# AuburnSounds/audio-formats

Measured on AMD Instinct MI355X. Metric: decoded samples/sec (batched MP3+OGG+FLAC) at 1/2/4/8 MI355X vs CPU ref, higher is better.
Workload: dtype f32 (MP3, Vorbis, CELT) + int32 (FLAC)

## Files before the change

audio-formats_amd/csrc/afg_api.hip:

```cpp
#include "afg_common.h"

#include <atomic>
#include <cstdlib>
#include <string>

namespace afg {

static thread_local char g_err[512] = "";

void set_error(const char *fmt, ...)
{
    va_list ap;
    va_start(ap, fmt);
    vsnprintf(g_err, sizeof(g_err), fmt, ap);
    va_end(ap);
}

int require_device()
{
    int n = 0;
    hipError_t e = hipGetDeviceCount(&n);
    if (e != hipSuccess || n <= 0) {
        set_error("no HIP device available (%s); this library has no CPU fallback",
                  e == hipSuccess ? "device count 0" : hipGetErrorString(e));
        return AFG_ERR_NO_DEVICE;
    }
    int dev = 0;
    AFG_HIP_CHECK(hipGetDevice(&dev));
    hipDeviceProp_t prop;
    AFG_HIP_CHECK(hipGetDeviceProperties(&prop, dev));
    if (std::strncmp(prop.gcnArchName, "gfx950", 6) != 0) {
        set_error("device %d is %s; kernels are built for gfx950 (MI355X) only", dev, prop.gcnArchName);
        return AFG_ERR_NO_DEVICE;
    }
    return AFG_OK;
}

int device_slot(int *dev, const char *who)
{
    *dev = 0;
    AFG_HIP_CHECK(hipGetDevice(dev));
    if (*dev < 0 || *dev >= AFG_MAX_DEVICES) {
        set_error("%s: device index %d does not fit this library's per-device tables (AFG_MAX_DEVICES = %d)", who, *dev,
                  AFG_MAX_DEVICES);
        return AFG_ERR_INVALID;
    }
    return AFG_OK;
}

static std::atomic<int> g_numeric_mode{ -1 };

int numeric_mode()
{
    const int m = g_numeric_mode.load(std::memory_order_relaxed);
    if (m >= 0) return m;
    const char *e = getenv("AFG_NUMERIC");
    if (e && !strcmp(e, "exact")) return AFG_NUMERIC_EXACT;
    return AFG_NUMERIC_TOLERANCE;
}

static std::atomic<long> g_dev_option[kDevCount] = { { -1 }, { -1 }, { -1 }, { -1 }, { -1 }, { -1 }, { -1 }, { -1 }, { -1 }, { -1 }, { -1 }, { -1 }, { -1 }, { -1 }, { -1 }, { -1 } };
static const char *const k_dev_option_name[kDevCount] = { "celt_path", "celt_de_seq", "celt_de_duo", "celt_seg_recs", "celt_whole_frames",
                                                          "vorbis_single", "mp3_chunks", "mp3_float_upload", "vorbis_host_floor",
                                                          "flac_host_res32", "vorbis_seg_packets", "batch_groups", "stage_chunk_samples", "resample_scratch_bytes",
                                                          "mel_scratch_bytes", "trim_scratch_bytes" };

long dev_option(DevOption which) { return g_dev_option[which].load(std::memory_order_relaxed); }

int DeviceArray::upload(const void *host, size_t nbytes)
{
    release();
    if (nbytes == 0) return AFG_OK;
    hipError_t e = hipMalloc(&ptr, nbytes);
    if (e != hipSuccess) {
        ptr = nullptr;
        set_error("hipMalloc(%zu) failed: %s", nbytes, hipGetErrorString(e));
        return e == hipErrorOutOfMemory ? AFG_ERR_OOM : AFG_ERR_HIP;
    }
    bytes = nbytes;
    AFG_HIP_CHECK(hipMemcpy(ptr, host, nbytes, hipMemcpyHostToDevice));
    return AFG_OK;
}

void DeviceArray::release()
{
    if (ptr && owned) (void)hipFree(ptr);
    ptr = nullptr;
    bytes = 0;
    owned = true;
}

}

extern "C" {

int afg_abi_version(void) { return AFG_ABI_VERSION; }

const char *afg_status_string(int status)
{
    switch (status) {
    case AFG_OK: return "ok";
    case AFG_ERR_INVALID: return "invalid argument";
    case AFG_ERR_NO_DEVICE: return "no usable gfx950 device";
    case AFG_ERR_HIP: return "HIP runtime error";
    case AFG_ERR_OOM: return "out of memory";
    case AFG_ERR_UNSUPPORTED: return "unsupported";
    default: return "unknown status";
    }
}

const char *afg_last_error(void) { return afg::g_err; }

int afg_get_numeric_mode(void) { return afg::numeric_mode(); }

int afg_dev_option(const char *name, int value)
{
    for (int i = 0; name && i < afg::kDevCount; i++)
        if (!strcmp(name, afg::k_dev_option_name[i])) {
            afg::g_dev_option[i].store(value < 0 ? -1 : value, std::memory_order_relaxed);
            return AFG_OK;
        }
    afg::set_error("afg_dev_option: no option named '%s'", name ? name : "(null)");
    return AFG_ERR_INVALID;
}

int afg_set_numeric_mode(int mode)
{
    if (mode != AFG_NUMERIC_EXACT && mode != AFG_NUMERIC_TOLERANCE && mode != AFG_NUMERIC_FROM_ENV) {
        afg::set_error("afg_set_numeric_mode: unknown mode %d", mode);
        return AFG_ERR_INVALID;
    }
    const int prev = afg::numeric_mode();
    afg::g_numeric_mode.store(mode, std::memory_order_relaxed);
    return prev;
}

int afg_device_count(void)
{
    int n = 0;
    hipError_t e = hipGetDeviceCount(&n);
    if (e != hipSuccess) {
        afg::set_error("hipGetDeviceCount failed: %s", hipGetErrorString(e));
        return e == hipErrorNoDevice ? 0 : AFG_ERR_HIP;
    }
    return n;
}

int afg_device_name(int device, char *buf, size_t buflen)
{
    if (!buf || buflen == 0) return AFG_ERR_INVALID;
    hipDeviceProp_t prop;
    AFG_HIP_CHECK(hipGetDeviceProperties(&prop, device));
    snprintf(buf, buflen, "%s (%s, %d CUs)", prop.name, prop.gcnArchName, prop.multiProcessorCount);
    return AFG_OK;
}

int afg_device_malloc(void **d_ptr, size_t bytes)
{
    if (!d_ptr) return AFG_ERR_INVALID;
    *d_ptr = nullptr;
    if (int rc = afg::require_device()) return rc;
    hipError_t e = hipMalloc(d_ptr, bytes ? bytes : 1);
    if (e != hipSuccess) {
        afg::set_error("hipMalloc(%zu) failed: %s", bytes, hipGetErrorString(e));
        return e == hipErrorOutOfMemory ? AFG_ERR_OOM : AFG_ERR_HIP;
    }
    return AFG_OK;
}

int afg_device_free(void *d_ptr)
{
    if (d_ptr) AFG_HIP_CHECK(hipFree(d_ptr));
    return AFG_OK;
}

int afg_memcpy_h2d(void *d_dst, const void *src, size_t bytes, void *hip_stream)
{
    AFG_HIP_CHECK(hipMemcpyAsync(d_dst, src, bytes, hipMemcpyHostToDevice, (hipStream_t)hip_stream));
    return AFG_OK;
}

int afg_memcpy_d2h(void *dst, const void *d_src, size_t bytes, void *hip_stream)
{
    AFG_HIP_CHECK(hipMemcpyAsync(dst, d_src, bytes, hipMemcpyDeviceToHost, (hipStream_t)hip_stream));
    return AFG_OK;
}

namespace {
typedef float probe_f4 __attribute__((ext_vector_type(4)));
__global__ __launch_bounds__(256) void copy_probe_kernel(const probe_f4 *__restrict__ in, probe_f4 *__restrict__ out, size_t n)
{
    const size_t i = (size_t)blockIdx.x * 256 + threadIdx.x;
    if (i < n) __builtin_nontemporal_store(__builtin_nontemporal_load(in + i), out + i);
}
}

namespace {
__global__ __launch_bounds__(256) void lds_fill_kernel(uint32_t word, uint32_t *sink)
{
    extern __shared__ uint32_t lds_words[];
    for (uint32_t i = threadIdx.x; i < 160u * 1024u / 4u; i += 256) lds_words[i] = word;
    __syncthreads();
    if (sink && lds_words[(threadIdx.x * 97u) % (160u * 1024u / 4u)] != word) *sink = 1;
}
}

int afg_lds_fill_probe_hip(uint32_t word, void *hip_stream)
{
    if (int rc = afg::require_device()) return rc;
    static uint32_t *sink = nullptr;
    if (!sink) AFG_HIP_CHECK(hipMalloc(&sink, 256));
    AFG_HIP_CHECK(hipFuncSetAttribute((const void *)lds_fill_kernel, hipFuncAttributeMaxDynamicSharedMemorySize, 160 * 1024));
    hipLaunchKernelGGL(lds_fill_kernel, dim3(256 * 16), dim3(256), 160 * 1024, (hipStream_t)hip_stream, word, sink);
    AFG_HIP_CHECK(hipGetLastError());
    return AFG_OK;
}

int afg_copy_probe_hip(void *d_dst, const void *d_src, size_t bytes, void *hip_stream)
{
    if (!d_dst || !d_src || (bytes & 15) || (((uintptr_t)d_dst | (uintptr_t)d_src) & 15)) {
        afg::set_error("afg_copy_probe_hip: pointers and size must be 16-byte aligned");
        return AFG_ERR_INVALID;
    }
    if (int rc = afg::require_device()) return rc;
    const size_t n = bytes / 16, blocks = (n + 255) / 256;
    if (blocks == 0) return AFG_OK;
    if (blocks > 0x7fffffffull) {
        afg::set_error("afg_copy_probe_hip: at most 2^31 blocks of 4 KiB per call");
        return AFG_ERR_INVALID;
    }
    hipLaunchKernelGGL(copy_probe_kernel, dim3((uint32_t)blocks), dim3(256), 0, (hipStream_t)hip_stream,
                       (const probe_f4 *)d_src, (probe_f4 *)d_dst, n);
    AFG_HIP_CHECK(hipGetLastError());
    return AFG_OK;
}

int afg_stream_synchronize(void *hip_stream)
{
    AFG_HIP_CHECK(hipStreamSynchronize((hipStream_t)hip_stream));
    return AFG_OK;
}

}
```

audio-formats_amd/csrc/afg_common.h:

```cpp
#pragma once
#include <hip/hip_runtime.h>
#include <cstdarg>
#include <cstdint>
#include <cstdio>
#include <cstring>

#include "../../include/afg.h"

namespace afg {

void set_error(const char *fmt, ...);

int require_device();

#define AFG_MAX_DEVICES 64
int device_slot(int *dev, const char *who);

int numeric_mode();

enum DevOption { kDevCeltPath, kDevCeltDeSeq, kDevCeltDeDuo, kDevCeltSegRecs, kDevCeltWholeFrames, kDevVorbisSingle,
                 kDevMp3Chunks, kDevMp3FloatUpload, kDevVorbisHostFloor, kDevFlacHostRes32, kDevVorbisSegPackets, kDevBatchGroups, kDevStageChunkSamples, kDevResampleScratchBytes, kDevMelScratchBytes, kDevTrimScratchBytes, kDevCount };
long dev_option(DevOption which);

#define AFG_HIP_CHECK(expr)                                                              \
    do {                                                                                 \
        hipError_t e__ = (expr);                                                         \
        if (e__ != hipSuccess) {                                                         \
            ::afg::set_error("%s failed: %s (%s:%d)", #expr, hipGetErrorString(e__),     \
                             __FILE__, __LINE__);                                        \
            return AFG_ERR_HIP;                                                          \
        }                                                                                \
    } while (0)

struct PlanArena {
    uint8_t *host = nullptr, *dev = nullptr;
    size_t cap = 0, used = 0;
    hipStream_t stream = nullptr;
};

int mp3_plan_create_at(afg_mp3_plan **plan, uint32_t n_streams, const uint32_t *granules, const uint8_t *channels,
                       const uint64_t *blk_base, uint32_t seg_granules, PlanArena *arena = nullptr);

void mp3_launch_tolerance(uint32_t n_segs, const void *d_segs, const void *d_streams, const float *d_coef,
                          const uint32_t *d_flags, float *d_pcm, float *d_state, hipStream_t stream);

int vorbis_plan_create_at(afg_vorbis_plan **plan, uint32_t n_streams, const uint32_t *packets, const uint8_t *channels,
                          const uint16_t *blocksize0, const uint16_t *blocksize1, const uint8_t *pflags,
                          const uint64_t *spec_base, uint32_t seg_packets);

int collate_launch(const afg_collate_span *h_spans, uint64_t n_spans, const afg_collate_span *d_spans, uint64_t n_tiles,
                   const float *d_in, uint64_t in_floats, float *d_out, uint64_t out_floats, hipStream_t stream);

int resample_launch(const afg_resample_row *h_rows, uint64_t n_rows, const afg_resample_row *d_rows, uint64_t n_tiles,
                    const float *d_in, uint64_t in_floats, const float *d_taps, uint64_t taps_floats, float *d_out,
                    uint64_t out_floats, hipStream_t stream);

int melspec_launch(const afg_mel_row *h_rows, uint64_t n_rows, const afg_mel_row *d_rows, uint64_t n_tiles, const afg_mel_params *params,
                   const float *d_in, uint64_t in_floats, const float *d_basis, uint64_t basis_floats, const float *d_filters,
                   uint64_t filters_floats, float *d_out, uint64_t out_floats, hipStream_t stream);

int melspec_fft_launch(const afg_mel_row *h_rows, uint64_t n_rows, const afg_mel_row *d_rows, uint64_t n_tiles, const afg_mel_params *params,
                       const float *d_in, uint64_t in_floats, const float *d_table, uint64_t table_floats, const float *d_filters,
                       uint64_t filters_floats, float *d_out, uint64_t out_floats, hipStream_t stream);
bool mel_fft_n_ok(uint32_t n_fft);

int normalize_launch(const afg_norm_group *h_groups, uint64_t n_groups, const afg_norm_group *d_groups, uint64_t n_tiles,
                     const afg_norm_params *params, const float *d_in, uint64_t in_floats, float *d_out, uint64_t out_floats,
                     void *d_partials, afg_norm_stats *d_stats, hipStream_t stream);

int cepstra_launch(const afg_cep_row *h_rows, uint64_t n_rows, const afg_cep_row *d_rows, uint64_t n_tiles, const afg_cep_params *params,
                   const float *d_in, uint64_t in_floats, const float *d_dct, uint64_t dct_floats, float *d_out, uint64_t out_floats,
                   hipStream_t stream);

int trim_launch(const afg_trim_group *h_groups, uint64_t n_groups, const afg_trim_group *d_groups, uint64_t n_blocks, uint64_t n_tiles,
                const afg_trim_params *params, const float *d_in, uint64_t in_floats, float *d_out, uint64_t out_floats, double *d_blocks,
                afg_trim_region *d_regions, hipStream_t stream);

struct DeviceArray {
    void *ptr = nullptr;
    size_t bytes = 0;
    bool owned = true;
    int upload(const void *host, size_t nbytes);
    void release();
};

}
```

audio-formats_amd/csrc/mp3_transform.hip:

```cpp
#define AFG_MP3_FMA 0
#define AFG_MP3_KERNEL mp3_transform_kernel
#include "mp3_kernel.h"

#include <vector>

struct afg_mp3_plan {
    uint32_t n_streams = 0;
    uint32_t n_segs = 0;
    uint64_t blocks = 0;
    afg::DeviceArray d_segs, d_streams;
};

extern "C" {

int afg_mp3_plan_create(afg_mp3_plan **plan, uint32_t n_streams, const uint32_t *granules,
                        const uint8_t *channels, uint32_t seg_granules)
{
    return afg::mp3_plan_create_at(plan, n_streams, granules, channels, nullptr, seg_granules);
}

}

int afg::mp3_plan_create_at(afg_mp3_plan **plan, uint32_t n_streams, const uint32_t *granules,
                            const uint8_t *channels, const uint64_t *blk_base, uint32_t seg_granules, afg::PlanArena *arena)
{
    if (!plan) return AFG_ERR_INVALID;
    *plan = nullptr;
    if (n_streams && (!granules || !channels)) {
        afg::set_error("afg_mp3_plan_create: NULL stream description");
        return AFG_ERR_INVALID;
    }
    if (int rc = afg::require_device()) return rc;
    if (seg_granules == 0) seg_granules = 48;

    std::vector<Mp3Stream> streams(n_streams);
    std::vector<Mp3Seg> segs;
    uint64_t blk = 0, extent = 0;
    for (uint32_t s = 0; s < n_streams; s++) {
        if (channels[s] != 1 && channels[s] != 2) {
            afg::set_error("afg_mp3_plan_create: stream %u has %u channels (1 or 2 expected)", s, channels[s]);
            return AFG_ERR_INVALID;
        }
        if (blk_base) blk = blk_base[s];
        streams[s] = Mp3Stream{ blk, granules[s], channels[s] };
        for (uint32_t g0 = 0; g0 < granules[s]; g0 += seg_granules) {
            uint32_t cnt = granules[s] - g0 < seg_granules ? granules[s] - g0 : seg_granules;
            segs.push_back(Mp3Seg{ s, g0, cnt, (g0 + cnt == granules[s]) ? 1u : 0u });
        }
        blk += (uint64_t)granules[s] * channels[s];
        extent = blk > extent ? blk : extent;
    }
    if (segs.size() > 0x7fffffffu) {
        afg::set_error("afg_mp3_plan_create: too many segments");
        return AFG_ERR_INVALID;
    }
    afg_mp3_plan *p = new (std::nothrow) afg_mp3_plan;
    if (!p) return AFG_ERR_OOM;
    p->n_streams = n_streams;
    p->n_segs = (uint32_t)segs.size();
    p->blocks = extent;
    int rc = AFG_OK;
    const size_t seg_bytes = segs.size() * sizeof(Mp3Seg), st_bytes = streams.size() * sizeof(Mp3Stream);
    if (arena && arena->used + seg_bytes + st_bytes <= arena->cap) {
        uint8_t *h = arena->host + arena->used, *d = arena->dev + arena->used;
        std::memcpy(h, segs.data(), seg_bytes);
        std::memcpy(h + seg_bytes, streams.data(), st_bytes);
        hipError_t e = hipMemcpyAsync(d, h, seg_bytes + st_bytes, hipMemcpyHostToDevice, arena->stream);
        if (e != hipSuccess) {
            afg::set_error("plan table upload failed: %s", hipGetErrorString(e));
            rc = AFG_ERR_HIP;
        }
        p->d_segs.ptr = d; p->d_segs.bytes = seg_bytes; p->d_segs.owned = false;
        p->d_streams.ptr = d + seg_bytes; p->d_streams.bytes = st_bytes; p->d_streams.owned = false;
        arena->used += (seg_bytes + st_bytes + 15) & ~(size_t)15;
    } else {
        rc = p->d_segs.upload(segs.data(), seg_bytes);
        if (!rc) rc = p->d_streams.upload(streams.data(), st_bytes);
    }
    if (rc) {
        afg_mp3_plan_destroy(p);
        return rc;
    }
    *plan = p;
    return AFG_OK;
}

extern "C" {

void afg_mp3_plan_destroy(afg_mp3_plan *plan)
{
    if (!plan) return;
    plan->d_segs.release();
    plan->d_streams.release();
    delete plan;
}

uint64_t afg_mp3_plan_blocks(const afg_mp3_plan *plan) { return plan ? plan->blocks : 0; }
uint32_t afg_mp3_plan_segments(const afg_mp3_plan *plan) { return plan ? plan->n_segs : 0; }

int afg_mp3_transform_hip(const afg_mp3_plan *plan, const float *d_coef, const uint32_t *d_flags,
                          float *d_pcm, float *d_state, void *hip_stream)
{
    if (!plan) return AFG_ERR_INVALID;
    if (plan->n_segs == 0) return AFG_OK;
    if (!d_coef || !d_flags || !d_pcm) {
        afg::set_error("afg_mp3_transform_hip: NULL device pointer");
        return AFG_ERR_INVALID;
    }
    if (afg::numeric_mode() == AFG_NUMERIC_TOLERANCE)
        afg::mp3_launch_tolerance(plan->n_segs, plan->d_segs.ptr, plan->d_streams.ptr, d_coef, d_flags, d_pcm, d_state, (hipStream_t)hip_stream);
    else
        hipLaunchKernelGGL(mp3_transform_kernel, dim3(plan->n_segs), dim3(64), 0, (hipStream_t)hip_stream,
                           (const Mp3Seg *)plan->d_segs.ptr, (const Mp3Stream *)plan->d_streams.ptr,
                           d_coef, d_flags, d_pcm, d_state);
    AFG_HIP_CHECK(hipGetLastError());
    return AFG_OK;
}

}
```

Baseline: 801.4 billion.

## Use occupancy-graded variable MP3 segment sizes sorted largest-first

Replaces the fixed 48-granule MP3 segmentation with segments whose length is derived from the total granule count and the number of resident wave slots (occupancy times CU count). Segment length starts large and shrinks toward a floor as work runs out, and the segments are then sorted largest-first so long blocks are dispatched early and short ones fill the tail. This is meant to cut launch tail imbalance and per-segment overhead. Longer segments carry more sequential state and give less parallelism when inputs are small, and the plan now does an occupancy query and a sort on the host.

```diff
diff --git a/audio-formats_amd/csrc/afg_api.hip b/audio-formats_amd/csrc/afg_api.hip
--- a/audio-formats_amd/csrc/afg_api.hip
+++ b/audio-formats_amd/csrc/afg_api.hip
@@ -59,11 +59,11 @@
     return AFG_NUMERIC_TOLERANCE;
 }
 
-static std::atomic<long> g_dev_option[kDevCount] = { { -1 }, { -1 }, { -1 }, { -1 }, { -1 }, { -1 }, { -1 }, { -1 }, { -1 }, { -1 }, { -1 }, { -1 }, { -1 }, { -1 }, { -1 }, { -1 } };
+static std::atomic<long> g_dev_option[kDevCount] = { { -1 }, { -1 }, { -1 }, { -1 }, { -1 }, { -1 }, { -1 }, { -1 }, { -1 }, { -1 }, { -1 }, { -1 }, { -1 }, { -1 }, { -1 }, { -1 }, { -1 } };
 static const char *const k_dev_option_name[kDevCount] = { "celt_path", "celt_de_seq", "celt_de_duo", "celt_seg_recs", "celt_whole_frames",
                                                           "vorbis_single", "mp3_chunks", "mp3_float_upload", "vorbis_host_floor",
                                                           "flac_host_res32", "vorbis_seg_packets", "batch_groups", "stage_chunk_samples", "resample_scratch_bytes",
-                                                          "mel_scratch_bytes", "trim_scratch_bytes" };
+                                                          "mel_scratch_bytes", "trim_scratch_bytes", "mp3_graded_slots" };
 
 long dev_option(DevOption which) { return g_dev_option[which].load(std::memory_order_relaxed); }
 
diff --git a/audio-formats_amd/csrc/afg_common.h b/audio-formats_amd/csrc/afg_common.h
--- a/audio-formats_amd/csrc/afg_common.h
+++ b/audio-formats_amd/csrc/afg_common.h
@@ -19,7 +19,8 @@
 int numeric_mode();
 
 enum DevOption { kDevCeltPath, kDevCeltDeSeq, kDevCeltDeDuo, kDevCeltSegRecs, kDevCeltWholeFrames, kDevVorbisSingle,
-                 kDevMp3Chunks, kDevMp3FloatUpload, kDevVorbisHostFloor, kDevFlacHostRes32, kDevVorbisSegPackets, kDevBatchGroups, kDevStageChunkSamples, kDevResampleScratchBytes, kDevMelScratchBytes, kDevTrimScratchBytes, kDevCount };
+                 kDevMp3Chunks, kDevMp3FloatUpload, kDevVorbisHostFloor, kDevFlacHostRes32, kDevVorbisSegPackets, kDevBatchGroups, kDevStageChunkSamples, kDevResampleScratchBytes, kDevMelScratchBytes, kDevTrimScratchBytes,
+                 kDevMp3GradedSlots, kDevCount };
 long dev_option(DevOption which);
 
 #define AFG_HIP_CHECK(expr)                                                              \
diff --git a/audio-formats_amd/csrc/graded_units.h b/audio-formats_amd/csrc/graded_units.h
--- /dev/null
+++ b/audio-formats_amd/csrc/graded_units.h
@@ -0,0 +1,35 @@
+#pragma once
+#include <algorithm>
+#include <cstdint>
+#include <vector>
+
+namespace afg {
+
+struct GradedUnits {
+    static constexpr uint64_t kRounds = 4, kGrade = 2;
+    uint32_t floor, cap, quantum;
+    uint64_t div, remaining;
+
+    GradedUnits(uint64_t total, uint64_t slots, uint32_t floor_, uint32_t cap_max, uint32_t quantum_)
+        : floor(floor_), quantum(quantum_), div((slots ? slots : 1) * kGrade), remaining(total)
+    {
+        const uint64_t c = total / ((slots ? slots : 1) * kRounds) / quantum * quantum;
+        cap = (uint32_t)std::min<uint64_t>(std::max<uint64_t>(c, floor), std::max(cap_max, floor));
+    }
+    uint32_t next(uint32_t left)
+    {
+        const uint64_t want = remaining / div / quantum * quantum;
+        const uint32_t len = (uint32_t)std::min<uint64_t>(std::max<uint64_t>(want, floor), cap);
+        const uint32_t cnt = left < len ? left : len;
+        remaining -= remaining < cnt ? remaining : cnt;
+        return cnt;
+    }
+};
+
+template <class Seg>
+void graded_sort(std::vector<Seg> &segs)
+{
+    std::stable_sort(segs.begin(), segs.end(), [](const Seg &a, const Seg &b) { return a.count > b.count; });
+}
+
+}
diff --git a/audio-formats_amd/csrc/mp3_transform.hip b/audio-formats_amd/csrc/mp3_transform.hip
--- a/audio-formats_amd/csrc/mp3_transform.hip
+++ b/audio-formats_amd/csrc/mp3_transform.hip
@@ -1,8 +1,37 @@
 #define AFG_MP3_FMA 0
 #define AFG_MP3_KERNEL mp3_transform_kernel
 #include "mp3_kernel.h"
+#include "graded_units.h"
 
+#include <mutex>
 #include <vector>
+
+#ifndef AFG_MP3_SEG_FLOOR
+#define AFG_MP3_SEG_FLOOR 48
+#endif
+#ifndef AFG_MP3_SEG_CAP
+#define AFG_MP3_SEG_CAP 256
+#endif
+
+namespace {
+
+uint32_t mp3_wave_slots()
+{
+    struct Dev { std::once_flag once; uint32_t slots = 0; };
+    static Dev state[AFG_MAX_DEVICES];
+    int dev = 0;
+    if (afg::device_slot(&dev, "afg_mp3_plan_create")) return 0;
+    std::call_once(state[dev].once, [&] {
+        int nb = 0, n_cu = 0, cur = 0;
+        if (hipGetDevice(&cur) != hipSuccess) return;
+        if (hipDeviceGetAttribute(&n_cu, hipDeviceAttributeMultiprocessorCount, cur) != hipSuccess) return;
+        if (hipOccupancyMaxActiveBlocksPerMultiprocessor(&nb, (const void *)mp3_transform_kernel, 64, 0) != hipSuccess) return;
+        if (nb > 0 && n_cu > 0) state[dev].slots = (uint32_t)nb * (uint32_t)n_cu;
+    });
+    return state[dev].slots;
+}
+
+}
 
 struct afg_mp3_plan {
     uint32_t n_streams = 0;
@@ -31,7 +60,15 @@
         return AFG_ERR_INVALID;
     }
     if (int rc = afg::require_device()) return rc;
-    if (seg_granules == 0) seg_granules = 48;
+    long slots = 0;
+    if (seg_granules == 0) {
+        slots = afg::dev_option(afg::kDevMp3GradedSlots);
+        if (slots < 0) slots = (long)mp3_wave_slots();
+        if (slots <= 0) seg_granules = 48;
+    }
+    uint64_t total = 0;
+    for (uint32_t s = 0; s < n_streams; s++) total += granules[s];
+    afg::GradedUnits graded(total, (uint64_t)slots, AFG_MP3_SEG_FLOOR, AFG_MP3_SEG_CAP, 8);
 
     std::vector<Mp3Stream> streams(n_streams);
     std::vector<Mp3Seg> segs;
@@ -43,13 +80,15 @@
         }
         if (blk_base) blk = blk_base[s];
         streams[s] = Mp3Stream{ blk, granules[s], channels[s] };
-        for (uint32_t g0 = 0; g0 < granules[s]; g0 += seg_granules) {
-            uint32_t cnt = granules[s] - g0 < seg_granules ? granules[s] - g0 : seg_granules;
+        for (uint32_t g0 = 0, cnt = 0; g0 < granules[s]; g0 += cnt) {
+            const uint32_t left = granules[s] - g0;
+            cnt = seg_granules ? (left < seg_granules ? left : seg_granules) : graded.next(left);
             segs.push_back(Mp3Seg{ s, g0, cnt, (g0 + cnt == granules[s]) ? 1u : 0u });
         }
         blk += (uint64_t)granules[s] * channels[s];
         extent = blk > extent ? blk : extent;
     }
+    if (!seg_granules) afg::graded_sort(segs);
     if (segs.size() > 0x7fffffffu) {
         afg::set_error("afg_mp3_plan_create: too many segments");
         return AFG_ERR_INVALID;
```

Result: no change. 796.4 billion (-0.6%).
